# 101001000/ElevenRender

Hardware: AMD Instinct MI355X
Metric: Msamples/sec (rays traced x bounces) at 1920x1080, 1M-tri scene (higher is better)
Workload: dtype f32; 1 GPU; C2: 1000000-triangle random soup + 2048x1024 sky HDRI, 1920x1080, max_bounces 8, 1 step = 1 spp pass (config total 256 spp), seed 12345; schedule=stream

## Files before the change

### elevenrender_amd/abi.py

```python
import ctypes as C
import os

import numpy as np

_HERE = os.path.dirname(os.path.abspath(__file__))
LIB_PATH = os.environ.get("ELEVEN_HIP_LIB") or os.path.join(_HERE, "libeleven_hip.so")

ER_OK = 0
ER_ERR_INVALID_ARG, ER_ERR_NO_DEVICE, ER_ERR_HIP, ER_ERR_STATE, ER_ERR_OOM = -1, -2, -3, -4, -5
PASS_BEAUTY, PASS_DENOISE, PASS_NORMAL, PASS_TANGENT, PASS_BITANGENT, PASS_COUNT = 0, 1, 2, 3, 4, 5
PASS_NAMES = {"beauty": 0, "denoise": 1, "normal": 2, "tangent": 3, "bitangent": 4}
FLAG_POINT_LIGHTS, FLAG_COUNTERS, FLAG_MEGAKERNEL, FLAG_PROFILE, FLAG_FUSED, FLAG_WAVEFRONT, FLAG_GPU_BUILD, FLAG_MIS, FLAG_STREAM = 1, 2, 4, 8, 16, 32, 64, 128, 256
FLAG_HOST_BUILD = 512
FLAG_MESH_LIGHTS = 1024
UPDATE_CAMERA, UPDATE_GEOMETRY = 1, 2
EDIT_CAMERA, EDIT_GEOMETRY, EDIT_MATERIALS, EDIT_TEXTURES, EDIT_HDRI = 1, 2, 4, 8, 16
REBUILD_NEVER, REBUILD_ALWAYS, REBUILD_AUTO = 0, 1, 2
TOPO_REMOVE, TOPO_APPEND = 1, 2
FEATURE_ALBEDO, FEATURE_DEPTH, FEATURE_COUNT = 0, 1, 2
FEATURE_NAMES = {"albedo": 0, "depth": 1}
ID_NONE, ID_SLOTS = 0xFFFFFFFF, 4
ID_TRIANGLE, ID_OBJECT, ID_MATERIAL, ID_KIND_COUNT = 0, 1, 2, 3
ID_KIND_NAMES = {"triangle": 0, "object": 1, "material": 2}

# ... 491 lines not shown
    "er_state_import": (C.c_int, [_P, _P, C.c_uint64]),
    "er_comm_unique_id": (C.c_int, [C.POINTER(C.c_uint8)]),
    "er_comm_create": (C.c_int, [C.POINTER(C.c_uint8), C.c_uint32, C.c_uint32, C.c_int, C.POINTER(_P)]),
    "er_comm_destroy": (None, [_P]),
    "er_gather_pass": (C.c_int, [_P, C.c_int, _P, C.c_uint32]),
    "er_debug_comm_create_local": (C.c_int, [C.c_uint32, C.POINTER(_P)]),
    "er_comm_create_local": (C.c_int, [C.c_uint32, C.POINTER(_P)]),
    "er_debug_stream_info": (C.c_int, [_P, C.POINTER(ErStreamInfo)]),
    "er_debug_gather_buffers": (C.c_int, [_P, C.c_uint32, C.POINTER(_P), C.POINTER(C.c_uint64), C.POINTER(_P), C.POINTER(C.c_uint64)]),
    "er_debug_comm_loopback": (C.c_int, [_P, C.c_uint64, C.POINTER(C.c_double)]),
    "er_measure_hbm_peak": (C.c_int, [C.c_int, C.c_uint64, C.c_uint32, _FP, _FP]),
    "er_debug_eval": (C.c_int, [_P, C.c_int, _FP, C.c_uint32, C.c_uint32, _FP, C.c_uint32]),
    "er_debug_trace_rays": (C.c_int, [_P, _FP, _FP, C.c_uint32, _IP, _FP, _IP, _IP, _FP, _FP, _IP]),
    "er_debug_trace_pixel": (C.c_int, [_P, C.c_uint32, C.POINTER(ErTraceRec), C.c_int, C.POINTER(C.c_int)]),
    "er_debug_read_light_table": (C.c_int, [_P, _IP, _FP, C.c_uint32]),
    "er_debug_set_host_alloc_limit": (None, [C.c_uint64]),
    "er_debug_set_gpu_build_failure": (None, [C.c_int]),
    "er_debug_closest_hit": (C.c_int, [_P, C.POINTER(C.c_float), C.POINTER(C.c_float), C.c_uint32, C.POINTER(C.c_int32), C.POINTER(C.c_float),
                                       C.POINTER(C.c_float)]),
}

_lib = None


class ErError(RuntimeError):
    def __init__(self, code, msg):
        super().__init__(f"eleven_hip error {code}: {msg}")
        self.code = code


# ... 151 lines not shown
```

### elevenrender_amd/csrc/er_api.cpp

```cpp
#include <algorithm>
#include <chrono>

#include "er_api_stages.h"
#include <thread>
#include <system_error>

using namespace erh;

int er_abi_version(void) { return ER_ABI_VERSION; }
const char* er_last_error(void) { return g_err.c_str(); }

int er_device_count(void) {
    int n = 0;
    if (hipGetDeviceCount(&n) != hipSuccess) return 0;
    return n;
}

static int er_device_info_impl(int index, ErDeviceInfo* out) {
    if (!out) return fail(ER_ERR_INVALID_ARG, "er_device_info: out is NULL");
    int n = er_device_count();
    if (index < 0 || index >= n) return fail(ER_ERR_NO_DEVICE, "er_device_info: no such HIP device");
    hipDeviceProp_t p;
    HIP_TRY(hipGetDeviceProperties(&p, index));
    memset(out, 0, sizeof(*out));
// ... 316 lines not shown
            o[0] = a[0];
            o[1] = A.channels == 1 ? a[0] : a[1];
            o[2] = A.channels == 1 ? a[0] : (A.channels == 2 ? 0.0f : a[2]);
            o[3] = powered && !r_done ? ermath::er_pow(r, 2.2f) : r;
            o[4] = powered && !k_done ? ermath::er_pow(mt, 2.2f) : mt;
        }
    }
    s->fused_any = P.fused_any;
    if ((rc = upload(s->d_mat_fused, fused.data(), fused.size(), s->stream)) != ER_OK) return rc;
    s->kept.hdri = P.hdri;
    if (!s->hdri_tex.data.empty()) memcpy(pool.data() + P.hdri.offset, s->hdri_tex.data.data(), s->hdri_tex.data.size() * sizeof(float));
    if ((rc = upload(s->d_textures, table.data(), table.size(), s->stream)) != ER_OK) return rc;
    if ((rc = upload(s->d_tex_pool, pool.data(), pool.size(), s->stream)) != ER_OK) return rc;
    s->tex_pool_cap = pool.size();
    if ((rc = upload(s->d_cdf, s->hdri_cdf.data(), s->hdri_cdf.size(), s->stream)) != ER_OK) return rc;
    s->kept.buckets = er_build_cdf_guide(s->hdri_cdf.data(), s->hdri_tex.width * s->hdri_tex.height, B.guide);
    return upload(s->d_guide, B.guide.data(), B.guide.size(), s->stream);
}

int begin_emitters(ErScene* s, BeginStaging& B, const char* who) {
    if (!(s->params.flags & ER_FLAG_MESH_LIGHTS)) return ER_OK;
    int rc;
    std::vector<int32_t>& etex = B.etex;
    for (const ErMaterial& m : s->materials)
        if (m.emission_tex >= 0 && (size_t)m.emission_tex < s->textures.size()) etex.push_back(m.emission_tex);
    std::sort(etex.begin(), etex.end());
    etex.erase(std::unique(etex.begin(), etex.end()), etex.end());
    ScopedDevBuf<int32_t> d_etex;
    if ((rc = upload(d_etex, etex.data(), etex.size(), s->stream)) != ER_OK) return rc;
    float* tab = nullptr;
    HIP_TRY(er_lights_build(s->d_nodes8.p + s->kept.accel.n8_pieces, s->d_attr.p, s->tri_count, s->d_materials.p, s->d_textures.p, s->d_tex_pool.p, d_etex.p,
                            (uint32_t)etex.size(), (uint32_t)s->textures.size(), &tab, &s->light_emitters, &s->light_total, s->stream));
// ... 106 lines not shown
    D.node8_count = g.nodes8_count;
    D.prune_margin = lift_bound + 1e-5f * scene_scale;
    D.max_lift = lift_bound;
    D.scene_scale = scene_scale;
    D.materials = s->d_materials.p;
    D.mat_pre = s->d_mat_pre.p;
    D.textures = s->d_textures.p;
    D.tex_pool = s->d_tex_pool.p;
    D.mat_fused = s->d_mat_fused.p;
    D.fused_any = s->fused_any ? 1u : 0u;
    D.hdri_tex = s->kept.hdri;
    D.hdri_cdf = s->d_cdf.p;
    D.hdri_guide = s->d_guide.p;
    D.hdri_buckets = s->kept.buckets;
    D.hdri_radiance_sum = s->hdri_radiance_sum;
    D.cam = s->camera;
    D.x_res = s->x_res;
    D.y_res = s->y_res;
    D.tiles_x = s->tiles_x();
    D.tiles_y = s->tiles_y();
    D.max_bounces = s->params.max_bounces;
    {
        auto pow2 = [](int32_t v) { return v > 0 && (v & (v - 1)) == 0; };
        bool all = pow2(s->kept.hdri.width) && pow2(s->kept.hdri.height);
        for (const HostTex& t : s->textures) all = all && pow2(t.width) && pow2(t.height);
        D.tex_pow2 = all ? 1u : 0u;
        if (const char* e = getenv("ER_TEX_POW2")) D.tex_pow2 = (atoi(e) != 0 && all) ? 1u : 0u;
    }
    D.trace_every_query = 0u;
    if (const char* e = getenv("ER_TRACE_EVERY_QUERY")) D.trace_every_query = atoi(e) != 0 ? 1u : 0u;
// ... 620 lines not shown
```

### elevenrender_amd/csrc/er_api_edit.cpp

```cpp
#include <algorithm>
#include <chrono>

#include "er_api_stages.h"
#include "er_topology_host.h"

using namespace erh;

static_assert(ER_TOPO_REMOVE == ER_TOPO_HOST_REMOVE && ER_TOPO_APPEND == ER_TOPO_HOST_APPEND, "er_topology_host.h restates the two bits");

static_assert(ER_EDIT_CAMERA == ER_UPDATE_CAMERA && ER_EDIT_GEOMETRY == ER_UPDATE_GEOMETRY, "an ErSceneUpdate's bits are the first two of an ErSceneEdit");

namespace {

const uint32_t LOOK_BITS = ER_EDIT_MATERIALS | ER_EDIT_TEXTURES | ER_EDIT_HDRI;

struct XformList {
    uint32_t count = 0;
    const ErObjectTransform* x = nullptr;
    std::vector<ErXformEntry> entries;
    uint32_t moved = 0;
};


int edit_refit(ErScene* s, bool new_normals, bool new_tangents, const ErSparseList* sp, const XformList* xf, const char* who) {
// ... 202 lines not shown
            s->d_tex_pool.release();
            s->d_tex_pool = bigger;
            s->tex_pool_cap = std::max<size_t>(need, 1);
        }
        if (!s->hdri_tex.data.empty())
            HIP_TRY(hipMemcpyAsync(s->d_tex_pool.p + head, s->hdri_tex.data.data(), s->hdri_tex.data.size() * sizeof(float), hipMemcpyHostToDevice, s->stream));
        HIP_TRY(hipEventRecord(ev.b, s->stream));
        HIP_TRY(hipStreamSynchronize(s->stream));
        (void)hipEventElapsedTime(&stage_ms, ev.a, ev.b);
        s->d_tex_pool.n = need;
        s->kept.hdri = DevTex{s->hdri_tex.width, s->hdri_tex.height, s->hdri_tex.channels, s->hdri_tex.filter, (uint32_t)head};
        stage = 1;
    }
    if (what & ER_EDIT_HDRI) {
        if ((rc = upload(s->d_cdf, s->hdri_cdf.data(), s->hdri_cdf.size(), s->stream)) != ER_OK) return rc;
        s->kept.buckets = er_build_cdf_guide(s->hdri_cdf.data(), s->hdri_tex.width * s->hdri_tex.height, B.guide);
        if ((rc = upload(s->d_guide, B.guide.data(), B.guide.size(), s->stream)) != ER_OK) return rc;
    }
    return ER_OK;
}

int edit_emitters(ErScene* s, BeginStaging& B, const char* who) {
    s->d_light_tab.release(); s->light_emitters = 0; s->light_total = 0.0f;
    return begin_emitters(s, B, who);
}

int edit_restart(ErScene* s, BeginStaging& B) {
    s->ad_on = false;
    s->rendered = 0;
    s->timing_open = false;
    s->prof_used = 0;
    s->profile = ErProfile{};
// ... 480 lines not shown
```

### elevenrender_amd/csrc/er_api_stages.h

```cpp
#pragma once
#include "er_scene.h"

namespace erh {

struct BeginStaging {
    ErBvhBuild bvh;
    std::vector<ErTriIsect> isect;
    std::vector<ErTriAttr> attr;
    std::vector<float4> geom, mat_pre;
    std::vector<DevTex> table;
    std::vector<float> pool;
    std::vector<DevFused> fused;
    std::vector<uint32_t> guide, owned;
    std::vector<int32_t> etex;
    StreamDeal deal;
};

inline int check_pool_floats(uint64_t floats, const char* who) {
    return floats >= (1ull << 32) ? fail(ER_ERR_INVALID_ARG, std::string(who) + ": texture pool exceeds 2^32 floats") : ER_OK;
}

int begin_accel(ErScene* s, BeginStaging& B, hipEvent_t built_ev, const char* who, const ErGpuSceneArrays* device_arrays = nullptr);
bool accel_device_first(const ErScene* s);
void accel_publish(ErScene* s, float up_ms);
int upload_materials(ErScene* s, BeginStaging& B);
void plan_of_scene(const ErScene* s, TexPlan& P);
int begin_emitters(ErScene* s, BeginStaging& B, const char* who);
int begin_render_state(ErScene* s, BeginStaging& B, hipEvent_t uploads_done);

}
```

### elevenrender_amd/csrc/er_bounce.inc

```
#ifndef ER_BOUNCE_FUSE
#define ER_BOUNCE_FUSE true
#endif
#ifndef ER_BOUNCE_SKIP_EQUAL
#define ER_BOUNCE_SKIP_EQUAL true
#endif
{
    const bool er_skip_equal = (ER_BOUNCE_SKIP_EQUAL) && S.trace_every_query == 0u;
    const int hw = S.hdri_tex.width, hh = S.hdri_tex.height;
    const bool er_mis = EXT && (S.ext_flags & ER_FLAG_MIS) != 0;
#ifdef ER_BOUNCE_MESH
    constexpr bool er_mesh = EXT && (ER_BOUNCE_MESH);
#else
    constexpr bool er_mesh = false;
#endif
    if (hslot < 0) {
        float u, v;
        spherical_mapping(-1 * ray.d, u, v);
        if (EXT) {
            F3 er_env = tex_filtered(S, S.hdri_tex, u, v);
            if (er_mis && prev_pdf >= 0.0f) {
                const float er_ph = hdri_pdf(S, ermath::f2i(u * hw), ermath::f2i(v * hh));
                er_env = er_env * (1.0f / (1.0f + er_ph / prev_pdf));
                if (COUNT) c_texels++;
            }
            light = light + reduction * er_env;
        } else {
            light = light + reduction * tex_filtered(S, S.hdri_tex, u, v);
        }
        if (COUNT) c_texels++;
        done = true;
    } else {
        c_shaded++;
        ER_TP(2);
        HitFull hit;
        full_hit(S, (uint32_t)hslot, ray, hit);
        const ErMaterial& mat = S.materials[hit.material];
        HitData hd;
        generate_hit_data<COUNT, ER_BOUNCE_FUSE>(S, mat, hit, hd, c_texels);
        int shader = mat.albedo_shader_id;
        if (shader != -1) {
            hd.albedo = f3s(0);
            if (shader >= 0 && shader < 4) hd.albedo = f3(1, 1, 0);
        }
        if (rng_next(rs) <= hd.opacity) {
            F3 wo = ray.d * -1.0f;
            F3 N = hd.normal;
            c_hdri++;
            ER_TP(3);
            int count = er_cdf_search(S.hdri_cdf, hw * hh, S.hdri_guide, S.hdri_buckets, rng_next(rs));
            const bool hw_pow2 = (hw & (hw - 1)) == 0 && hw > 0 && count >= 0;
            float tcx = (float)(hw_pow2 ? (int)((unsigned)count & (unsigned)(hw - 1)) : count % hw);
            float tcy = (float)(hw_pow2 ? (int)((unsigned)count >> (31 - __builtin_clz((unsigned)hw))) : count / hw);
            float d1 = rng_next(rs), d2 = rng_next(rs), d3 = rng_next(rs);
            const bool er_lights = EXT && !er_mesh && (S.ext_flags & ER_FLAG_POINT_LIGHTS) != 0 && S.light_count > 0;
            float er_rl = 0.0f;
            if (er_lights) er_rl = rng_next(rs);
            float er_mp = 0.0f, er_mu1 = 0.0f, er_mu2 = 0.0f;
            if (er_mesh) { er_mp = rng_next(rs); er_mu1 = rng_next(rs); er_mu2 = rng_next(rs); }
            ER_TP(4);
            F3 wibrdf = DisneySample(hd, wo, N, d1, d2, d3);
            float nu = tcx / (float)hw, nv = tcy / (float)hh;
            float iu, iv;
            inverse_transform_uv(S.hdri_tex, nu, nv, iu, iv);
            F3 wihdri = normalized(reverse_spherical_mapping(iu, iv)) * -1.0f;
            F3 hdriValue = tex_uv(S, S.hdri_tex, iu, iv);
            if (COUNT) c_texels += 2;
            F3 evalh = DisneyEval(hd, wo, N, wihdri);
            float hdripdf = hdri_pdf(S, ermath::f2i(iu * hw), ermath::f2i(iv * hh));
            float absdot = __builtin_fabsf(dot(wihdri, N));
            float er_wnee = 1.0f;
            if (er_mis) er_wnee = 1.0f / (1.0f + DisneyPdf(hd, wo, N, wihdri) / hdripdf);
            F3 er_em = hd.emission;
            if (er_mesh && prev_pdf >= 0.0f) {
                const float er_ph = mesh_prob(S)[hslot];
                if (er_ph > 0.0f) {
                    F3 er_a, er_b, er_c, er_ng;
                    float er_area;
                    mesh_tri(S, (uint32_t)hslot, er_a, er_b, er_c, er_ng, er_area);
                    const float er_dh = mesh_d + length(hit.position - ray.o);
                    const float er_pl = er_ph * (er_dh * er_dh) / (er_area * __builtin_fabsf(dot(er_ng, ray.d)));
                    er_em = er_em * (1.0f / (1.0f + er_pl / prev_pdf));
                }
            }
// ... 65 lines not shown
                        const float er_lpdf = mesh_prob(S)[er_k] * (er_dist * er_dist) / (er_area * __builtin_fabsf(er_cosl));
                        const float er_wl = 1.0f / (1.0f + DisneyPdf(hd, wo, N, er_dir) / er_lpdf);
                        const F3 er_ml = er_le * er_evall * __builtin_fabsf(dot(er_dir, N)) / er_lpdf * er_wl;
                        const F3 er_lv = reduction * er_ml, er_lo = reduction * f3s(0);
                        if (er_skip_equal && !pending && same_bits(er_lv, er_lo)) {
                            light = light + er_lv;
                        } else {
                            const Ray er_lr = make_ray(hd.position + er_dir * 0.001f, er_dir);
                            ER_BOUNCE_LIGHT_QUERY(er_lr, (int)er_k, length(er_p - er_lr.o), er_lv, er_lo);
                            lpending = true;
                        }
                    }
                }
            }
            ER_TP(5);
            float brdfpdf = DisneyPdf(hd, wo, N, wibrdf);
            reduction = reduction * (DisneyEval(hd, wo, N, wibrdf) * __builtin_fabsf(dot(wibrdf, N)) / brdfpdf);
            if (er_mis || er_mesh) prev_pdf = brdfpdf;
            if (bounce == 0) { ER_BOUNCE_FIRST_HIT(hd.normal, hd.tangent, hd.bitangent); }
            ray = make_ray(hit.position + wibrdf * 0.001f, wibrdf);
            if (er_mesh) mesh_d = 0.001f;
        } else {
            if (er_mesh) mesh_d = mesh_d + length(hit.position - ray.o) + 0.001f;
            ray = make_ray(hit.position + ray.d * 0.001f, ray.d);
        }
        ER_TP(6);
        bounce++;
        if (bounce >= S.max_bounces) done = true;
    }
}
```

### elevenrender_amd/csrc/er_debug.hip

```cpp
#include "er_debug.h"

#include "er_device.h"
#include "er_shade.h"
#include "er_trav.h"

using namespace erd;

__global__ __launch_bounds__(64) void er_debug_trace_kernel(DevScene S, const float* __restrict__ o, const float* __restrict__ d, uint32_t n,
                                                             const int32_t* __restrict__ self, const float* __restrict__ limit,
                                                             int32_t* __restrict__ tri_out, int32_t* __restrict__ slot_out, float* __restrict__ pos_out,
                                                             float* __restrict__ dist_out, int32_t* __restrict__ info_out, uint2* spill_base) {
    __shared__ uint2 s_stack[WF_LDS_STACK * 64];
    __shared__ int s_stack2[ER_STACK * 64];
    const uint32_t i = blockIdx.x * 64 + threadIdx.x;
    if (i >= n) return;
    uint2* stack = s_stack + threadIdx.x;
    uint2* spill = spill_base + (size_t)blockIdx.x * (ER_STACK8 * 64) + threadIdx.x;
    int* stack2 = s_stack2 + threadIdx.x;
    Ray ray;
    ray.o = f3(o[3 * i], o[3 * i + 1], o[3 * i + 2]);
    ray.d = f3(d[3 * i], d[3 * i + 1], d[3 * i + 2]);
    unsigned cn = 0, ct = 0;
    int info = 0;
    if (self) {
// ... 75 lines not shown
            const int cs_ = trav_run_closest<false>(S, s_stack, spill, s_stack2, (sr), __builtin_inff(), info_, c_nodes, c_tris);     \
            rec->shadow_tri = cs_ < 0 ? -1 : __builtin_bit_cast(int, S.tri_isect[(size_t)cs_ * 3].w);                                 \
        }                                                                                                                             \
    }
#define ER_BOUNCE_LIGHT_QUERY(lr, self_slot, limit, lv, lo)                                                                          \
    {                                                                                                                                 \
        int info_;                                                                                                                    \
        c_rays++;                                                                                                                     \
        const bool occ_ = trav_run_shadow<false>(S, s_stack, spill, s_stack2, (lr), (self_slot), (limit), info_, c_nodes, c_tris);    \
        light = light + (occ_ ? (lo) : (lv));                                                                                         \
        if (rec) rec->light_occ = occ_ ? 1 : 0;                                                                                       \
    }
#define ER_BOUNCE_FIRST_HIT(n, t, b) aov_n = (n); aov_t = (t); aov_b = (b)
#define ER_BOUNCE_MESH MESH
#define ER_BOUNCE_SKIP_EQUAL false
#include "er_bounce.inc"
#undef ER_BOUNCE_HDRI_QUERY
#undef ER_BOUNCE_LIGHT_QUERY
#undef ER_BOUNCE_FIRST_HIT
#undef ER_BOUNCE_MESH
#undef ER_BOUNCE_SKIP_EQUAL
        (void)pending; (void)lpending; (void)traced;
        if (rec) {
            uint32_t r1 = rs_before;
            (void)rng_next(r1);
            rec->opaque = (hslot >= 0 && rs != r1) ? 1 : 0;
            if (hslot >= 0) { rec->wi[0] = ray.d.x; rec->wi[1] = ray.d.y; rec->wi[2] = ray.d.z; }
            rec->light[0] = light.x; rec->light[1] = light.y; rec->light[2] = light.z;
            rec->reduction[0] = reduction.x; rec->reduction[1] = reduction.y; rec->reduction[2] = reduction.z;
        }
        if (done) break;
    }
    const uint32_t sa = S.samples[idx];
    const uint32_t sa2 = accumulate_sample(S, idx, sa, light, aov_n, aov_t, aov_b);
    if (sa2 != sa) S.samples[idx] = sa2;
    S.rng[idx] = rs;
// ... 150 lines not shown
```

### elevenrender_amd/csrc/er_debug_api.cpp

```cpp
#include "er_scene.h"
#include "er_debug.h"

using namespace erh;

#include "../../include/eleven_hip_debug.h"

static int er_debug_closest_hit_impl(ErScene* s, const float* origins, const float* dirs, uint32_t n, int32_t* tri_ids, float* positions, float* distances) {
    if (!s || !origins || !dirs || !tri_ids || !positions || !distances) return fail(ER_ERR_INVALID_ARG, "er_debug_closest_hit: NULL argument");
    std::lock_guard<std::mutex> lk(s->mtx);
    if (!s->begun) return fail(ER_ERR_STATE, "er_debug_closest_hit: er_render_begin has not succeeded");
    HIP_TRY(hipSetDevice(s->device));
    ScopedDevBuf<float> d_o, d_d, d_pos, d_dist;
    ScopedDevBuf<int32_t> d_tri;
    int rc;
    if ((rc = upload(d_o, origins, (size_t)n * 3, s->stream)) != ER_OK) return rc;
    if ((rc = upload(d_d, dirs, (size_t)n * 3, s->stream)) != ER_OK) return rc;
    if ((rc = upload(d_pos, (const float*)nullptr, (size_t)n * 3, s->stream)) != ER_OK) return rc;
    if ((rc = upload(d_dist, (const float*)nullptr, (size_t)n, s->stream)) != ER_OK) return rc;
    if ((rc = upload(d_tri, (const int32_t*)nullptr, (size_t)n, s->stream)) != ER_OK) return rc;
    er_launch_debug_hit(s->dev, d_o.p, d_d.p, n, d_tri.p, d_pos.p, d_dist.p, s->stream);
    HIP_TRY(hipGetLastError());
    HIP_TRY(hipMemcpyAsync(tri_ids, d_tri.p, (size_t)n * 4, hipMemcpyDeviceToHost, s->stream));
    HIP_TRY(hipMemcpyAsync(positions, d_pos.p, (size_t)n * 12, hipMemcpyDeviceToHost, s->stream));
    HIP_TRY(hipMemcpyAsync(distances, d_dist.p, (size_t)n * 4, hipMemcpyDeviceToHost, s->stream));
// ... 355 lines not shown
    if (m == 0) return ER_OK;
    HIP_TRY(hipSetDevice(s->device));
    ScopedDevBuf<int32_t> d_tri;
    ScopedDevBuf<float> d_cdf;
    int rc;
    if ((rc = upload(d_tri, (const int32_t*)nullptr, m, s->stream)) != ER_OK) return rc;
    if ((rc = upload(d_cdf, (const float*)nullptr, m, s->stream)) != ER_OK) return rc;
    er_launch_light_table_read(s->dev.tri_isect, s->d_light_tab.p, s->tri_count, s->light_emitters, m, d_tri.p, d_cdf.p, s->stream);
    HIP_TRY(hipGetLastError());
    if (tri_index) HIP_TRY(hipMemcpyAsync(tri_index, d_tri.p, sizeof(int32_t) * m, hipMemcpyDeviceToHost, s->stream));
    if (cdf) HIP_TRY(hipMemcpyAsync(cdf, d_cdf.p, sizeof(float) * m, hipMemcpyDeviceToHost, s->stream));
    HIP_TRY(hipStreamSynchronize(s->stream));
    return ER_OK;
}

static int er_debug_eval_impl(ErScene* s, int kind, const float* in, uint32_t n, uint32_t in_stride, float* out, uint32_t out_stride) {
    static const uint32_t need_in[ER_FN_COUNT] = {1, 7, 7, 29, 29, 29, 3, 2, 4, 1, 2, 3};
    static const uint32_t need_out[ER_FN_COUNT] = {32, 6, 18, 3, 1, 3, 2, 3, 3, 1, 1, 1};
    if (!s || !in || !out) return fail(ER_ERR_INVALID_ARG, "er_debug_eval: NULL argument");
    if (kind < 0 || kind >= ER_FN_COUNT) return fail(ER_ERR_INVALID_ARG, "er_debug_eval: unknown kind");
    if (in_stride < need_in[kind] || out_stride < need_out[kind]) return fail(ER_ERR_INVALID_ARG, "er_debug_eval: stride smaller than the kind's item");
    std::lock_guard<std::mutex> lk(s->mtx);
    if (!s->begun) return fail(ER_ERR_STATE, "er_debug_eval: er_render_begin has not succeeded");
    if (kind == ER_FN_TEXTURE)
        for (uint32_t i = 0; i < n; i++) {
            int32_t id;
            memcpy(&id, &in[(size_t)i * in_stride], 4);
            if (id < -1 || id >= (int32_t)s->textures.size()) return fail(ER_ERR_INVALID_ARG, "er_debug_eval: texture id out of range");
            if (id >= 0 && (size_t)id < s->tex_mode.size() && s->tex_mode[(size_t)id] != 0)
                return fail(ER_ERR_STATE, "er_debug_eval: texture " + std::to_string(id) + " is kept compacted on the device (first channel" +
// ... 110 lines not shown
    return guarded("er_debug_accel_cost_host", [&]() -> int {
        return er_debug_accel_cost_host_impl(nodes8, node8_count, node8_pieces, isect, tri_count, sums, node_terms, node_cap, tri_terms, tri_cap);
    });
}
int er_debug_bvh_check(const float* vertices, const float* normals, uint32_t tri_count, int threads, ErBvhCheck* out) { return guarded("er_debug_bvh_check", [&]() -> int { return er_debug_bvh_check_impl(vertices, normals, tri_count, threads, out); }); }
int er_debug_trace_rays(ErScene* s, const float* origins, const float* dirs, uint32_t n, const int32_t* self_slots, const float* limits, int32_t* tri_ids,
                        int32_t* slots, float* positions, float* distances, int32_t* info) {
    return guarded("er_debug_trace_rays", [&]() -> int { return er_debug_trace_rays_impl(s, origins, dirs, n, self_slots, limits, tri_ids, slots, positions, distances, info); });
}
int er_debug_trace_pixel(ErScene* s, uint32_t idx, ErTraceRec* recs, int max_recs, int* count) {
    return guarded("er_debug_trace_pixel", [&]() -> int { return er_debug_trace_pixel_impl(s, idx, recs, max_recs, count); });
}
int er_debug_read_light_table(ErScene* s, int32_t* tri_index, float* cdf, uint32_t cap) {
    return guarded("er_debug_read_light_table", [&]() -> int { return er_debug_read_light_table_impl(s, tri_index, cdf, cap); });
}
int er_debug_eval(ErScene* s, int kind, const float* in, uint32_t n, uint32_t in_stride, float* out, uint32_t out_stride) {
    return guarded("er_debug_eval", [&]() -> int { return er_debug_eval_impl(s, kind, in, n, in_stride, out, out_stride); });
}
int er_measure_hbm_peak(int device, uint64_t bytes, uint32_t iters, float* copy_GBps, float* read_GBps) {
    return guarded("er_measure_hbm_peak", [&]() -> int { return er_measure_hbm_peak_impl(device, bytes, iters, copy_GBps, read_GBps); });
}
int er_debug_transform_apply(const float* m, uint32_t count, const float* v, const float* n, const float* t, float* ov, float* on, float* ot) {
    return guarded("er_debug_transform_apply", [&]() -> int {
        if (!m || (count && (!v || !n || !t || !ov || !on || !ot))) return fail(ER_ERR_INVALID_ARG, "er_debug_transform_apply: NULL argument");
        if (!er_xform_apply(m, count, v, n, t, ov, on, ot)) return fail(ER_ERR_INVALID_ARG, "er_debug_transform_apply: a matrix entry is not finite, or det(L) is not > 0");
        return ER_OK;
    });
}
int er_debug_id_rank(const uint32_t* ids, uint32_t count, uint32_t* out_ids, uint32_t* out_counts, uint32_t* distinct) {
    return guarded("er_debug_id_rank", [&]() -> int {
// ... 8 lines not shown
```

### elevenrender_amd/csrc/er_device.h

```cpp
#pragma once
#include <hip/hip_runtime.h>
#include <stdint.h>

#include "../../include/eleven_hip.h"
#include "er_bvh.h"
#include "er_cdf.h"
#include "er_math.h"

#ifdef ER_ISA_MARKS
#define ER_MARK(name) asm volatile("; ER_MARK " name ::: "memory")
#else
#define ER_MARK(name) ((void)0)
#endif

#ifndef ER_TP
#define ER_TP(n) ((void)0)
#endif

#define ER_TILE 8
#define ER_STACK ER_BVH_MAX_DEPTH

struct DevTex {
    int32_t width, height, channels, filter;
    uint32_t offset;
// ... 36 lines not shown
    uint32_t tex_pow2;
    float cam_cx, cam_sx, cam_cy, cam_sy, cam_cz, cam_sz;
    uint32_t cam_trig_valid;
    uint32_t trace_every_query;
    uint32_t ext_flags;
    union { const ErPointLight* lights; const float* mesh_lights; };
    union { uint32_t light_count; uint32_t emitter_count; };
    float4* passes;
    uint32_t* samples;
    uint32_t* rng;
    const uint32_t* owned_tiles;
    uint32_t owned_tile_count;
    DevCounters* counters;
    uint32_t* tile_cost;
    uint32_t* px_draws;
};

__host__ __device__ __forceinline__ size_t er_pass_index(size_t npx, int pass, size_t idx) {
    return pass == ER_PASS_DENOISE ? 4 * npx + idx : idx * 4 + (size_t)(pass == ER_PASS_BEAUTY ? 0 : pass - 1);
}


namespace erd {

#define ERD __device__ __forceinline__

const float PIF = 3.14159265358979323846f;

struct F3 { float x, y, z; };
ERD F3 f3(float x, float y, float z) { F3 r; r.x = x; r.y = y; r.z = z; return r; }
// ... 12 lines not shown
ERD float dot(F3 a, F3 b) { return a.x * b.x + a.y * b.y + a.z * b.z; }
ERD F3 cross(F3 a, F3 b) {
    return f3((a.y * b.z - a.z * b.y), -(a.x * b.z - a.z * b.x), (a.x * b.y - a.y * b.x));
}
ERD float length(F3 a) { return __builtin_sqrtf(a.x * a.x + a.y * a.y + a.z * a.z); }
ERD F3 normalized(F3 a) {
    float l = length(a);
    if (l == 0) return a;
    return a / l;
}
ERD float clampf(float a, float b, float c) { return a < b ? b : a > c ? c : a; }
ERD float lerpf(float a, float b, float c) { return a + c * (b - a); }
ERD F3 lerpv(F3 a, F3 b, float c) { return f3(lerpf(a.x, b.x, c), lerpf(a.y, b.y, c), lerpf(a.z, b.z, c)); }
ERD float minf(float a, float b) { return a < b ? a : b; }
ERD float maxf(float a, float b) { return a > b ? a : b; }
ERD void limitUV(float& u, float& v) {
    u += (float)(-(int)(u > 1) + -(int)(u < 0));
    v += (float)(-(int)(v > 1) + -(int)(v < 0));
}

struct Ray { F3 o, d; };
ERD Ray make_ray(F3 o, F3 d) {
    Ray r;
    r.o = o;
    float l = length(d);
    if (l != 0) { d.x /= l; d.y /= l; d.z /= l; }
    r.d = d;
    return r;
}

ERD uint32_t jenkins_u32(uint32_t seed) {
// ... 284 lines not shown
        fused_coords(S, t, ermath::f2i(t2x), ermath::f2i(t2y), a4, r4);
        alb = lerpv(lerpv(a1, a2, a), lerpv(a3, a4, a), b);
        rm = lerpv(lerpv(r1, r2, a), lerpv(r3, r4, a), b);
    } else {
        fused_coords(S, t, ermath::f2i(u * t.width), ermath::f2i(v * t.height), alb, rm);
    }
}
ERD void spherical_mapping(F3 point, float& u, float& v) {
    F3 p = (point - f3s(0)) / 1.0f;
    float theta = ermath::er_acos(-p.y);
    float phi = ermath::er_atan2(-p.z, p.x) + PIF;
    u = phi / (2 * PIF);
    v = theta / PIF;
    limitUV(u, v);
}
ERD void inverse_transform_uv(const DevTex& t, float u, float v, float& nu, float& nv) {
    int x = ermath::f2i(u * t.width);
    int y = ermath::f2i(v * t.height);
    nu = (float)x / (float)t.width;
    nv = (float)y / (float)t.height;
    limitUV(nu, nv);
}
ERD F3 reverse_spherical_mapping(float u, float v) {
    float phi = u * 2 * PIF;
    float theta = v * PIF;
    float px = ermath::er_cos(phi - PIF);
    float py = -ermath::er_cos(theta);
    float pz = -ermath::er_sin(phi - PIF);
    float a = __builtin_sqrtf(1 - py * py);
    return f3(a * px, py, a * pz);
}

ERD int hdri_binary_search(const float* arr, float value, int length) {
    int from = 0;
    int to = length - 1;
    while (to - from > 0) {
        int m = from + (to - from) / 2;
        if (m >= length || m < 0) return 0;
        float am = arr[m];
        if (value == am) return m;
        if (value < am) to = m - 1;
        if (value > am) from = m + 1;
    }
    return to;
}
ERD float hdri_pdf(const DevScene& S, int x, int y) {
    F3 dv = tex_coords(S, S.hdri_tex, x, y);
    float theta = (((float)y / (float)S.hdri_tex.height)) * PIF;
    return ((dv.x + dv.y + dv.z) / S.hdri_radiance_sum) * S.hdri_tex.width * S.hdri_tex.height / (2.0f * PIF * ermath::er_sin(theta));
}

struct HitData {
    float metallic, roughness, clearcoatGloss, clearcoat, anisotropic, transmission, specular,
        specularTint, sheenTint, subsurface, sheen, opacity;
    float gtr1_log;
    F3 emission, albedo;
    F3 position, normal, tangent, bitangent;
};

ERD float SchlickFresnel(float u) {
    float m = clampf(1.0f - u, 0.0f, 1.0f);
    float m2 = m * m;
    return m2 * m2 * m;
}
// ... 159 lines not shown
```

### elevenrender_amd/csrc/er_scene.h

```cpp
#pragma once
#include <hip/hip_runtime.h>

#include <atomic>
#include <cmath>
#include <cstdio>
#include <cstdlib>
#include <cstring>
#include <map>
#include <set>
#include <memory>
#include <mutex>
#include <new>
#include <string>
#include <vector>

#include "../../include/eleven_hip.h"
#include "er_bvh.h"
#include "er_devbuf.h"
#include "er_device.h"
#include "er_gpu_build.h"
#include "er_kernels.h"
#include "er_wavefront.h"
#include "er_stream.h"
#include "er_stream_host.h"
// ... 116 lines not shown

    bool begun = false;
    int device = 0;
    ErRenderParams params{};
    hipStream_t stream = nullptr;
    hipEvent_t ev_start = nullptr, ev_stop = nullptr;
    bool timing_open = false;
    DevScene dev{};
    ErAccelInfo accel{};
    float accel_lo[3] = {0, 0, 0}, accel_hi[3] = {0, 0, 0};
    uint32_t accel_depth2 = 0;
    struct Kept {
        ErGpuBvhDevice accel;
        DevTex hdri{};
        int buckets = 0;
        uint32_t cus = 0, flags = 0;
    } kept;
    ErRefitTopo refit_topo;
    ErUpdateInfo upd{};
    ErEditInfo edit{};
    ErSparseInfo sparse{};
    ErObjectTable objects;
    ErXformDev xform_dev;
    ErSparseInfo xform{};
    uint32_t xform_objects = 0;
    ErGeomStore store;
    ErTopologyInfo topo{};
    void flush_poses() noexcept { er_objects_flush(objects, vertices.data(), normals.data(), tangents.data()); }
    uint64_t accel_version = 0, cost_version = ~0ull;
    ErAccelCost cost_kept{};
// ... 186 lines not shown
```

### elevenrender_amd/csrc/er_shade.h

```cpp
#pragma once
#include "er_device.h"

namespace erd {

static inline bool er_mesh_active(const DevScene& S) { return (S.ext_flags & ER_FLAG_MESH_LIGHTS) != 0; }
static inline bool er_ext_active(const DevScene& S) {
    return (S.ext_flags & ER_FLAG_MIS) != 0 || ((S.ext_flags & ER_FLAG_POINT_LIGHTS) != 0 && S.light_count > 0) || er_mesh_active(S);
}

ERD const float* mesh_prob(const DevScene& S) { return S.mesh_lights; }
ERD const float* mesh_cdf(const DevScene& S) { return S.mesh_lights + S.tri_count; }
ERD uint32_t mesh_slot(const DevScene& S, uint32_t k) { return __builtin_bit_cast(uint32_t, S.mesh_lights[(size_t)S.tri_count + S.emitter_count + k]); }
ERD uint32_t mesh_pick(const DevScene& S, float r) {
    const float* cdf = mesh_cdf(S);
    uint32_t lo = 0, hi = S.emitter_count;
    while (lo < hi) {
        const uint32_t m = lo + ((hi - lo) >> 1);
        if (cdf[m] > r) hi = m; else lo = m + 1;
    }
    return lo < S.emitter_count ? lo : S.emitter_count - 1;
}
ERD void mesh_tri(const DevScene& S, uint32_t slot, F3& v0, F3& v1, F3& v2, F3& ng, float& area) {
    float4 a, b, c;
    load_verts(S, slot, v0, v1, v2, a, b, c);
// ... 29 lines not shown
```

### elevenrender_amd/render.py

```python
import ctypes as C
from dataclasses import dataclass

import numpy as np

from . import abi, topology as topo


@dataclass
class RenderParameters:
    width: int = 1280
    height: int = 720
    sampleTarget: int = 100
    denoise: bool = False
    device: str = ""
    block_size: int = 8
    max_bounces: int = 5
    rank: int = 0
    world: int = 1
    flags: int = 0


@dataclass
class RenderInfo:
    samples: int = 0
# ... 332 lines not shown
        return {n: getattr(a, n) for n, _ in abi.ErAdaptiveInfo._fields_}

    def light_info(self):
        li = abi.ErLightInfo()
        abi.check(self.lib.er_light_info(self.handle, C.byref(li)))
        return {n: getattr(li, n) for n, _ in abi.ErLightInfo._fields_}

    def debug_light_table(self):
        n = self.light_info()["emitters"]
        tri = np.zeros(n, np.int32)
        cdf = np.zeros(n, np.float32)
        if n:
            abi.check(self.lib.er_debug_read_light_table(self.handle, tri.ctypes.data_as(C.POINTER(C.c_int32)), cdf.ctypes.data_as(C.POINTER(C.c_float)), n))
        return tri, cdf

    def tile_state(self):
        tx, ty = (self.scene.x_res + 7) // 8, (self.scene.y_res + 7) // 8
        err = np.empty((ty, tx), np.float32)
        spp = np.empty((ty, tx), np.uint32)
        abi.check(self.lib.er_read_tile_state(self.handle, err.ctypes.data_as(C.POINTER(C.c_float)), spp.ctypes.data_as(C.POINTER(C.c_uint32))))
        return err, spp

    def denoise(self, levels=0, colour_sigma=0.0):
        abi.check(self.lib.er_denoise(self.handle, levels, colour_sigma))

    def render_features(self, n=0):
        abi.check(self.lib.er_render_features(self.handle, n))

    def get_feature(self, name):
        f = abi.FEATURE_NAMES[str(name).lower()]
# ... 221 lines not shown
```

### include/eleven_hip_debug.h

```cpp
#ifndef ELEVEN_HIP_DEBUG_H
#define ELEVEN_HIP_DEBUG_H
#include <stdint.h>
#ifdef __cplusplus
extern "C" {
#endif

typedef struct ErBvhCheck {
    uint32_t node_count, leaf_count, max_depth, max_leaf_size;
    uint32_t tris_in_leaves;
    uint32_t duplicate_tris;
    uint32_t uncontained;
    uint32_t unreachable_nodes;
    float lift_bound;
    float build_ms;
    double sah_cost;
} ErBvhCheck;

int er_debug_bvh_check(const float* vertices, const float* normals, uint32_t tri_count, int threads, ErBvhCheck* out);

typedef struct ErAccelDump {
    uint32_t tri_count;
    uint32_t node_count;
    uint32_t node8_count;
    uint32_t node8_pieces;
// ... 33 lines not shown
    int32_t bounce;
    int32_t tri;
    int32_t shadow_tri;
    int32_t opaque;
    float position[3];
    float wi[3];
    float light[3];
    float reduction[3];
    int32_t shadow_occ;
    int32_t light_occ;
} ErTraceRec;

int er_debug_trace_pixel(struct ErScene* scene, uint32_t idx, ErTraceRec* recs, int max_recs, int* count);

int er_debug_read_light_table(struct ErScene* scene, int32_t* tri_index, float* cdf, uint32_t cap);

enum { ER_FN_RNG = 0, ER_FN_CAMERA_RAY, ER_FN_TRI_HIT, ER_FN_DISNEY_EVAL, ER_FN_DISNEY_PDF, ER_FN_DISNEY_SAMPLE, ER_FN_SPHERICAL,
       ER_FN_REV_SPHERICAL, ER_FN_TEXTURE, ER_FN_HDRI_SEARCH, ER_FN_HDRI_PDF, ER_FN_MATH, ER_FN_COUNT };
int er_debug_eval(struct ErScene* scene, int kind, const float* in, uint32_t n, uint32_t in_stride, float* out, uint32_t out_stride);

struct ErComm;
int er_debug_comm_create_local(uint32_t world, struct ErComm** out);

typedef struct ErStreamInfo {
    uint32_t waves, tracers;
    uint32_t large_regions;
    uint32_t deal_pending;
    uint32_t launches;
    uint32_t pixels_per_cu;
    double lanes_busy;
// ... 92 lines not shown
```

Measured before the change: 2109 Msamples/s.

## Precompute HDRI per-row/column trig tables and skip BRDF sampling on last bounce

Adds a small device table of per-column (cos/sin of phi, texel index) and per-row (cos theta, sqrt, sine pdf) values for the HDRI. NEE light sampling and the MIS pdf now look these up instead of evaluating sin/cos per sample. It also reuses the sampled HDRI texel value for the pdf instead of fetching it twice. A third change skips DisneySample, DisneyPdf, DisneyEval and the next-ray setup on the final bounce, since that ray is never traced. The costs are an extra table load per sample and slightly different float paths.

```diff
diff --git a/elevenrender_amd/abi.py b/elevenrender_amd/abi.py
--- a/elevenrender_amd/abi.py
+++ b/elevenrender_amd/abi.py
@@ -529,6 +529,8 @@
     "er_debug_trace_rays": (C.c_int, [_P, _FP, _FP, C.c_uint32, _IP, _FP, _IP, _IP, _FP, _FP, _IP]),
     "er_debug_trace_pixel": (C.c_int, [_P, C.c_uint32, C.POINTER(ErTraceRec), C.c_int, C.POINTER(C.c_int)]),
     "er_debug_read_light_table": (C.c_int, [_P, _IP, _FP, C.c_uint32]),
+    "er_debug_read_hdri_trig": (C.c_int, [_P, _UP, C.c_uint32, _UP, C.c_uint32]),
+    "er_debug_hdri_trig_host": (C.c_int, [C.c_int32, C.c_int32, _UP, _UP]),
     "er_debug_set_host_alloc_limit": (None, [C.c_uint64]),
     "er_debug_set_gpu_build_failure": (None, [C.c_int]),
     "er_debug_closest_hit": (C.c_int, [_P, C.POINTER(C.c_float), C.POINTER(C.c_float), C.c_uint32, C.POINTER(C.c_int32), C.POINTER(C.c_float),
diff --git a/elevenrender_amd/csrc/er_api.cpp b/elevenrender_amd/csrc/er_api.cpp
--- a/elevenrender_amd/csrc/er_api.cpp
+++ b/elevenrender_amd/csrc/er_api.cpp
@@ -354,8 +354,19 @@
     if ((rc = upload(s->d_tex_pool, pool.data(), pool.size(), s->stream)) != ER_OK) return rc;
     s->tex_pool_cap = pool.size();
     if ((rc = upload(s->d_cdf, s->hdri_cdf.data(), s->hdri_cdf.size(), s->stream)) != ER_OK) return rc;
+    return upload_hdri_guide(s, B);
+}
+
+int upload_hdri_guide(ErScene* s, BeginStaging& B) {
+    int rc;
     s->kept.buckets = er_build_cdf_guide(s->hdri_cdf.data(), s->hdri_tex.width * s->hdri_tex.height, B.guide);
-    return upload(s->d_guide, B.guide.data(), B.guide.size(), s->stream);
+    const size_t at = (B.guide.size() + 3) & ~(size_t)3;
+    B.guide.resize(at + erd::hdri_trig_words(s->kept.hdri.width, s->kept.hdri.height), 0u);
+    if ((rc = upload(s->d_guide, B.guide.data(), B.guide.size(), s->stream)) != ER_OK) return rc;
+    s->kept.trig_at = at;
+    er_launch_hdri_trig(s->kept.hdri, s->d_guide.p + at, s->stream);
+    HIP_TRY(hipGetLastError());
+    return ER_OK;
 }
 
 int begin_emitters(ErScene* s, BeginStaging& B, const char* who) {
@@ -492,6 +503,7 @@
     D.hdri_guide = s->d_guide.p;
     D.hdri_buckets = s->kept.buckets;
     D.hdri_radiance_sum = s->hdri_radiance_sum;
+    D.hdri_trig = getenv("ER_HDRI_TRIG_ON_DEVICE") ? nullptr : s->d_guide.p + s->kept.trig_at;
     D.cam = s->camera;
     D.x_res = s->x_res;
     D.y_res = s->y_res;
diff --git a/elevenrender_amd/csrc/er_api_edit.cpp b/elevenrender_amd/csrc/er_api_edit.cpp
--- a/elevenrender_amd/csrc/er_api_edit.cpp
+++ b/elevenrender_amd/csrc/er_api_edit.cpp
@@ -240,8 +240,7 @@
     }
     if (what & ER_EDIT_HDRI) {
         if ((rc = upload(s->d_cdf, s->hdri_cdf.data(), s->hdri_cdf.size(), s->stream)) != ER_OK) return rc;
-        s->kept.buckets = er_build_cdf_guide(s->hdri_cdf.data(), s->hdri_tex.width * s->hdri_tex.height, B.guide);
-        if ((rc = upload(s->d_guide, B.guide.data(), B.guide.size(), s->stream)) != ER_OK) return rc;
+        if ((rc = upload_hdri_guide(s, B)) != ER_OK) return rc;
     }
     return ER_OK;
 }
diff --git a/elevenrender_amd/csrc/er_api_stages.h b/elevenrender_amd/csrc/er_api_stages.h
--- a/elevenrender_amd/csrc/er_api_stages.h
+++ b/elevenrender_amd/csrc/er_api_stages.h
@@ -1,5 +1,6 @@
 #pragma once
 #include "er_scene.h"
+#include "er_hdri_trig.h"
 
 namespace erh {
 
@@ -24,6 +25,7 @@
 bool accel_device_first(const ErScene* s);
 void accel_publish(ErScene* s, float up_ms);
 int upload_materials(ErScene* s, BeginStaging& B);
+int upload_hdri_guide(ErScene* s, BeginStaging& B);
 void plan_of_scene(const ErScene* s, TexPlan& P);
 int begin_emitters(ErScene* s, BeginStaging& B, const char* who);
 int begin_render_state(ErScene* s, BeginStaging& B, hipEvent_t uploads_done);
diff --git a/elevenrender_amd/csrc/er_bounce.inc b/elevenrender_amd/csrc/er_bounce.inc
--- a/elevenrender_amd/csrc/er_bounce.inc
+++ b/elevenrender_amd/csrc/er_bounce.inc
@@ -3,6 +3,9 @@
 #endif
 #ifndef ER_BOUNCE_SKIP_EQUAL
 #define ER_BOUNCE_SKIP_EQUAL true
+#endif
+#ifndef ER_BOUNCE_KEEP_LAST
+#define ER_BOUNCE_KEEP_LAST false
 #endif
 {
     const bool er_skip_equal = (ER_BOUNCE_SKIP_EQUAL) && S.trace_every_query == 0u;
@@ -19,7 +22,9 @@
         if (EXT) {
             F3 er_env = tex_filtered(S, S.hdri_tex, u, v);
             if (er_mis && prev_pdf >= 0.0f) {
-                const float er_ph = hdri_pdf(S, ermath::f2i(u * hw), ermath::f2i(v * hh));
+                const int er_mx = ermath::f2i(u * hw), er_my = ermath::f2i(v * hh);
+                const float er_ms = (S.hdri_trig != nullptr && (unsigned)er_my < (unsigned)hh) ? hdri_trig_rows(S)[er_my].sin_row : hdri_pdf_sine(S.hdri_tex, er_my);
+                const float er_ph = hdri_pdf_of(S, tex_coords(S, S.hdri_tex, er_mx, er_my), er_ms);
                 er_env = er_env * (1.0f / (1.0f + er_ph / prev_pdf));
                 if (COUNT) c_texels++;
             }
@@ -49,8 +54,9 @@
             ER_TP(3);
             int count = er_cdf_search(S.hdri_cdf, hw * hh, S.hdri_guide, S.hdri_buckets, rng_next(rs));
             const bool hw_pow2 = (hw & (hw - 1)) == 0 && hw > 0 && count >= 0;
-            float tcx = (float)(hw_pow2 ? (int)((unsigned)count & (unsigned)(hw - 1)) : count % hw);
-            float tcy = (float)(hw_pow2 ? (int)((unsigned)count >> (31 - __builtin_clz((unsigned)hw))) : count / hw);
+            const int er_cx = hw_pow2 ? (int)((unsigned)count & (unsigned)(hw - 1)) : count % hw;
+            const int er_cy = hw_pow2 ? (int)((unsigned)count >> (31 - __builtin_clz((unsigned)hw))) : count / hw;
+            float tcx = (float)er_cx, tcy = (float)er_cy;
             float d1 = rng_next(rs), d2 = rng_next(rs), d3 = rng_next(rs);
             const bool er_lights = EXT && !er_mesh && (S.ext_flags & ER_FLAG_POINT_LIGHTS) != 0 && S.light_count > 0;
             float er_rl = 0.0f;
@@ -58,15 +64,30 @@
             float er_mp = 0.0f, er_mu1 = 0.0f, er_mu2 = 0.0f;
             if (er_mesh) { er_mp = rng_next(rs); er_mu1 = rng_next(rs); er_mu2 = rng_next(rs); }
             ER_TP(4);
-            F3 wibrdf = DisneySample(hd, wo, N, d1, d2, d3);
-            float nu = tcx / (float)hw, nv = tcy / (float)hh;
-            float iu, iv;
-            inverse_transform_uv(S.hdri_tex, nu, nv, iu, iv);
-            F3 wihdri = normalized(reverse_spherical_mapping(iu, iv)) * -1.0f;
-            F3 hdriValue = tex_uv(S, S.hdri_tex, iu, iv);
+            const bool er_last = !(ER_BOUNCE_KEEP_LAST) && bounce + 1u >= S.max_bounces;
+            F3 wibrdf = f3s(0);
+            if (!er_last) wibrdf = DisneySample(hd, wo, N, d1, d2, d3);
+            float er_px, er_pz, er_py, er_a, er_sin;
+            int er_ix, er_iy;
+            if (S.hdri_trig != nullptr && (unsigned)count < (unsigned)(hw * hh)) {
+                const HdriCol er_c = hdri_trig_cols(S)[er_cx];
+                const HdriRow er_r = hdri_trig_rows(S)[er_cy];
+                er_px = er_c.px; er_pz = er_c.pz; er_ix = er_c.ix;
+                er_py = er_r.py; er_a = er_r.a; er_iy = er_r.iy; er_sin = er_r.sin_pdf;
+            } else {
+                float nu = tcx / (float)hw, nv = tcy / (float)hh;
+                float iu, iv;
+                inverse_transform_uv(S.hdri_tex, nu, nv, iu, iv);
+                rsm_column(iu, er_px, er_pz);
+                rsm_row(iv, er_py, er_a);
+                er_ix = ermath::f2i(iu * hw); er_iy = ermath::f2i(iv * hh);
+                er_sin = hdri_pdf_sine(S.hdri_tex, er_iy);
+            }
+            F3 wihdri = normalized(f3(er_a * er_px, er_py, er_a * er_pz)) * -1.0f;
+            F3 hdriValue = tex_coords(S, S.hdri_tex, er_ix, er_iy);
             if (COUNT) c_texels += 2;
             F3 evalh = DisneyEval(hd, wo, N, wihdri);
-            float hdripdf = hdri_pdf(S, ermath::f2i(iu * hw), ermath::f2i(iv * hh));
+            float hdripdf = hdri_pdf_of(S, hdriValue, er_sin);
             float absdot = __builtin_fabsf(dot(wihdri, N));
             float er_wnee = 1.0f;
             if (er_mis) er_wnee = 1.0f / (1.0f + DisneyPdf(hd, wo, N, wihdri) / hdripdf);
@@ -162,11 +183,13 @@
                 }
             }
             ER_TP(5);
-            float brdfpdf = DisneyPdf(hd, wo, N, wibrdf);
-            reduction = reduction * (DisneyEval(hd, wo, N, wibrdf) * __builtin_fabsf(dot(wibrdf, N)) / brdfpdf);
-            if (er_mis || er_mesh) prev_pdf = brdfpdf;
+            if (!er_last) {
+                float brdfpdf = DisneyPdf(hd, wo, N, wibrdf);
+                reduction = reduction * (DisneyEval(hd, wo, N, wibrdf) * __builtin_fabsf(dot(wibrdf, N)) / brdfpdf);
+                if (er_mis || er_mesh) prev_pdf = brdfpdf;
+                ray = make_ray(hit.position + wibrdf * 0.001f, wibrdf);
+            }
             if (bounce == 0) { ER_BOUNCE_FIRST_HIT(hd.normal, hd.tangent, hd.bitangent); }
-            ray = make_ray(hit.position + wibrdf * 0.001f, wibrdf);
             if (er_mesh) mesh_d = 0.001f;
         } else {
             if (er_mesh) mesh_d = mesh_d + length(hit.position - ray.o) + 0.001f;
diff --git a/elevenrender_amd/csrc/er_debug.hip b/elevenrender_amd/csrc/er_debug.hip
--- a/elevenrender_amd/csrc/er_debug.hip
+++ b/elevenrender_amd/csrc/er_debug.hip
@@ -113,12 +113,14 @@
 #define ER_BOUNCE_FIRST_HIT(n, t, b) aov_n = (n); aov_t = (t); aov_b = (b)
 #define ER_BOUNCE_MESH MESH
 #define ER_BOUNCE_SKIP_EQUAL false
+#define ER_BOUNCE_KEEP_LAST true
 #include "er_bounce.inc"
 #undef ER_BOUNCE_HDRI_QUERY
 #undef ER_BOUNCE_LIGHT_QUERY
 #undef ER_BOUNCE_FIRST_HIT
 #undef ER_BOUNCE_MESH
 #undef ER_BOUNCE_SKIP_EQUAL
+#undef ER_BOUNCE_KEEP_LAST
         (void)pending; (void)lpending; (void)traced;
         if (rec) {
             uint32_t r1 = rs_before;
diff --git a/elevenrender_amd/csrc/er_debug_api.cpp b/elevenrender_amd/csrc/er_debug_api.cpp
--- a/elevenrender_amd/csrc/er_debug_api.cpp
+++ b/elevenrender_amd/csrc/er_debug_api.cpp
@@ -1,5 +1,6 @@
 #include "er_scene.h"
 #include "er_debug.h"
+#include "er_hdri_trig.h"
 
 using namespace erh;
 
@@ -393,6 +394,29 @@
     return ER_OK;
 }
 
+static int er_debug_read_hdri_trig_impl(ErScene* s, uint32_t* cols, uint32_t col_cap, uint32_t* rows, uint32_t row_cap) {
+    if (!s) return fail(ER_ERR_INVALID_ARG, "er_debug_read_hdri_trig: NULL scene");
+    std::lock_guard<std::mutex> lk(s->mtx);
+    if (!s->begun) return fail(ER_ERR_STATE, "er_debug_read_hdri_trig: er_render_begin has not succeeded");
+    const DevTex& t = s->kept.hdri;
+    const size_t nc = std::min<size_t>(col_cap, (size_t)std::max(t.width, 0)), nr = std::min<size_t>(row_cap, (size_t)std::max(t.height, 0));
+    HIP_TRY(hipSetDevice(s->device));
+    const uint32_t* tab = s->d_guide.p + s->kept.trig_at;
+    if (cols && nc) HIP_TRY(hipMemcpyAsync(cols, tab, nc * sizeof(erd::HdriCol), hipMemcpyDeviceToHost, s->stream));
+    if (rows && nr) HIP_TRY(hipMemcpyAsync(rows, tab + erd::hdri_trig_row_offset(t.width), nr * sizeof(erd::HdriRow), hipMemcpyDeviceToHost, s->stream));
+    HIP_TRY(hipStreamSynchronize(s->stream));
+    return ER_OK;
+}
+
+static int er_debug_hdri_trig_host_impl(int32_t width, int32_t height, uint32_t* cols, uint32_t* rows) {
+    if (width < 0 || height < 0 || (width && !cols) || (height && !rows)) return fail(ER_ERR_INVALID_ARG, "er_debug_hdri_trig_host: bad argument");
+    std::vector<uint32_t> tab(erd::hdri_trig_words(width, height));
+    er_hdri_trig_host(DevTex{width, height, 3, 0, 0u}, tab.data());
+    if (width) memcpy(cols, tab.data(), (size_t)width * sizeof(erd::HdriCol));
+    if (height) memcpy(rows, tab.data() + erd::hdri_trig_row_offset(width), (size_t)height * sizeof(erd::HdriRow));
+    return ER_OK;
+}
+
 static int er_debug_eval_impl(ErScene* s, int kind, const float* in, uint32_t n, uint32_t in_stride, float* out, uint32_t out_stride) {
     static const uint32_t need_in[ER_FN_COUNT] = {1, 7, 7, 29, 29, 29, 3, 2, 4, 1, 2, 3};
     static const uint32_t need_out[ER_FN_COUNT] = {32, 6, 18, 3, 1, 3, 2, 3, 3, 1, 1, 1};
@@ -533,6 +557,12 @@
 int er_debug_read_light_table(ErScene* s, int32_t* tri_index, float* cdf, uint32_t cap) {
     return guarded("er_debug_read_light_table", [&]() -> int { return er_debug_read_light_table_impl(s, tri_index, cdf, cap); });
 }
+int er_debug_read_hdri_trig(ErScene* s, uint32_t* cols, uint32_t col_cap, uint32_t* rows, uint32_t row_cap) {
+    return guarded("er_debug_read_hdri_trig", [&]() -> int { return er_debug_read_hdri_trig_impl(s, cols, col_cap, rows, row_cap); });
+}
+int er_debug_hdri_trig_host(int32_t width, int32_t height, uint32_t* cols, uint32_t* rows) {
+    return guarded("er_debug_hdri_trig_host", [&]() -> int { return er_debug_hdri_trig_host_impl(width, height, cols, rows); });
+}
 int er_debug_eval(ErScene* s, int kind, const float* in, uint32_t n, uint32_t in_stride, float* out, uint32_t out_stride) {
     return guarded("er_debug_eval", [&]() -> int { return er_debug_eval_impl(s, kind, in, n, in_stride, out, out_stride); });
 }
diff --git a/elevenrender_amd/csrc/er_device.h b/elevenrender_amd/csrc/er_device.h
--- a/elevenrender_amd/csrc/er_device.h
+++ b/elevenrender_amd/csrc/er_device.h
@@ -74,6 +74,7 @@
     DevCounters* counters;
     uint32_t* tile_cost;
     uint32_t* px_draws;
+    const uint32_t* hdri_trig;
 };
 
 __host__ __device__ __forceinline__ size_t er_pass_index(size_t npx, int pass, size_t idx) {
@@ -116,7 +117,7 @@
 ERD F3 lerpv(F3 a, F3 b, float c) { return f3(lerpf(a.x, b.x, c), lerpf(a.y, b.y, c), lerpf(a.z, b.z, c)); }
 ERD float minf(float a, float b) { return a < b ? a : b; }
 ERD float maxf(float a, float b) { return a > b ? a : b; }
-ERD void limitUV(float& u, float& v) {
+__host__ __device__ __forceinline__ void limitUV(float& u, float& v) {
     u += (float)(-(int)(u > 1) + -(int)(u < 0));
     v += (float)(-(int)(v > 1) + -(int)(v < 0));
 }
@@ -431,20 +432,27 @@
     v = theta / PIF;
     limitUV(u, v);
 }
-ERD void inverse_transform_uv(const DevTex& t, float u, float v, float& nu, float& nv) {
+__host__ __device__ __forceinline__ void inverse_transform_uv(const DevTex& t, float u, float v, float& nu, float& nv) {
     int x = ermath::f2i(u * t.width);
     int y = ermath::f2i(v * t.height);
     nu = (float)x / (float)t.width;
     nv = (float)y / (float)t.height;
     limitUV(nu, nv);
 }
+__host__ __device__ __forceinline__ void rsm_column(float u, float& px, float& pz) {
+    float phi = u * 2 * PIF;
+    px = ermath::er_cos(phi - PIF);
+    pz = -ermath::er_sin(phi - PIF);
+}
+__host__ __device__ __forceinline__ void rsm_row(float v, float& py, float& a) {
+    float theta = v * PIF;
+    py = -ermath::er_cos(theta);
+    a = __builtin_sqrtf(1 - py * py);
+}
 ERD F3 reverse_spherical_mapping(float u, float v) {
-    float phi = u * 2 * PIF;
-    float theta = v * PIF;
-    float px = ermath::er_cos(phi - PIF);
-    float py = -ermath::er_cos(theta);
-    float pz = -ermath::er_sin(phi - PIF);
-    float a = __builtin_sqrtf(1 - py * py);
+    float px, py, pz, a;
+    rsm_column(u, px, pz);
+    rsm_row(v, py, a);
     return f3(a * px, py, a * pz);
 }
 
@@ -461,10 +469,16 @@
     }
     return to;
 }
+__host__ __device__ __forceinline__ float hdri_pdf_sine(const DevTex& t, int y) {
+    float theta = (((float)y / (float)t.height)) * PIF;
+    return ermath::er_sin(theta);
+}
+ERD float hdri_pdf_of(const DevScene& S, F3 dv, float sin_theta) {
+    return ((dv.x + dv.y + dv.z) / S.hdri_radiance_sum) * S.hdri_tex.width * S.hdri_tex.height / (2.0f * PIF * sin_theta);
+}
 ERD float hdri_pdf(const DevScene& S, int x, int y) {
     F3 dv = tex_coords(S, S.hdri_tex, x, y);
-    float theta = (((float)y / (float)S.hdri_tex.height)) * PIF;
-    return ((dv.x + dv.y + dv.z) / S.hdri_radiance_sum) * S.hdri_tex.width * S.hdri_tex.height / (2.0f * PIF * ermath::er_sin(theta));
+    return hdri_pdf_of(S, dv, hdri_pdf_sine(S.hdri_tex, y));
 }
 
 struct HitData {
diff --git a/elevenrender_amd/csrc/er_hdri_trig.h b/elevenrender_amd/csrc/er_hdri_trig.h
--- /dev/null
+++ b/elevenrender_amd/csrc/er_hdri_trig.h
@@ -0,0 +1,50 @@
+#pragma once
+#include "er_device.h"
+
+namespace erd {
+
+struct HdriCol {
+    float px, pz;
+    int32_t ix;
+    float iu;
+};
+struct HdriRow {
+    float py, a;
+    int32_t iy;
+    float sin_pdf;
+    float iv;
+    float sin_row;
+};
+static_assert(sizeof(HdriCol) == 16 && sizeof(HdriRow) == 24, "er_hdri_trig.h: table entry sizes");
+
+#define ER_HT_HD __host__ __device__ __forceinline__
+
+ER_HT_HD HdriCol hdri_col_entry(const DevTex& t, int x) {
+    HdriCol c;
+    float nu = (float)x / (float)t.width, iv;
+    inverse_transform_uv(t, nu, 0.0f, c.iu, iv);
+    rsm_column(c.iu, c.px, c.pz);
+    c.ix = ermath::f2i(c.iu * t.width);
+    return c;
+}
+ER_HT_HD HdriRow hdri_row_entry(const DevTex& t, int y) {
+    HdriRow r;
+    float nv = (float)y / (float)t.height, iu;
+    inverse_transform_uv(t, 0.0f, nv, iu, r.iv);
+    rsm_row(r.iv, r.py, r.a);
+    r.iy = ermath::f2i(r.iv * t.height);
+    r.sin_pdf = hdri_pdf_sine(t, r.iy);
+    r.sin_row = hdri_pdf_sine(t, y);
+    return r;
+}
+
+ER_HT_HD size_t hdri_trig_row_offset(int width) { return (size_t)(width > 0 ? width : 0) * 4; }
+ER_HT_HD size_t hdri_trig_words(int width, int height) { return hdri_trig_row_offset(width) + (size_t)(height > 0 ? height : 0) * 6; }
+
+__device__ __forceinline__ const HdriCol* hdri_trig_cols(const DevScene& S) { return (const HdriCol*)S.hdri_trig; }
+__device__ __forceinline__ const HdriRow* hdri_trig_rows(const DevScene& S) { return (const HdriRow*)(S.hdri_trig + hdri_trig_row_offset(S.hdri_tex.width)); }
+
+}
+
+void er_launch_hdri_trig(const DevTex& t, uint32_t* table, hipStream_t stream);
+void er_hdri_trig_host(const DevTex& t, uint32_t* table);
diff --git a/elevenrender_amd/csrc/er_hdri_trig.hip b/elevenrender_amd/csrc/er_hdri_trig.hip
--- /dev/null
+++ b/elevenrender_amd/csrc/er_hdri_trig.hip
@@ -0,0 +1,26 @@
+#include "er_hdri_trig.h"
+
+using namespace erd;
+
+__global__ __launch_bounds__(64) void er_hdri_trig_kernel(DevTex t, uint32_t* __restrict__ table) {
+    const int w = t.width > 0 ? t.width : 0, h = t.height > 0 ? t.height : 0;
+    const int i = (int)(blockIdx.x * 64u + threadIdx.x);
+    if (i < w) {
+        ((HdriCol*)table)[i] = hdri_col_entry(t, i);
+    } else if (i - w < h) {
+        ((HdriRow*)(table + hdri_trig_row_offset(t.width)))[i - w] = hdri_row_entry(t, i - w);
+    }
+}
+
+void er_launch_hdri_trig(const DevTex& t, uint32_t* table, hipStream_t stream) {
+    const long long n = (long long)(t.width > 0 ? t.width : 0) + (long long)(t.height > 0 ? t.height : 0);
+    if (n == 0) return;
+    hipLaunchKernelGGL(er_hdri_trig_kernel, dim3((unsigned)((n + 63) / 64)), dim3(64), 0, stream, t, table);
+}
+
+void er_hdri_trig_host(const DevTex& t, uint32_t* table) {
+    HdriCol* cols = (HdriCol*)table;
+    HdriRow* rows = (HdriRow*)(table + hdri_trig_row_offset(t.width));
+    for (int x = 0; x < t.width; x++) cols[x] = hdri_col_entry(t, x);
+    for (int y = 0; y < t.height; y++) rows[y] = hdri_row_entry(t, y);
+}
diff --git a/elevenrender_amd/csrc/er_scene.h b/elevenrender_amd/csrc/er_scene.h
--- a/elevenrender_amd/csrc/er_scene.h
+++ b/elevenrender_amd/csrc/er_scene.h
@@ -154,6 +154,7 @@
         ErGpuBvhDevice accel;
         DevTex hdri{};
         int buckets = 0;
+        size_t trig_at = 0;
         uint32_t cus = 0, flags = 0;
     } kept;
     ErRefitTopo refit_topo;
diff --git a/elevenrender_amd/csrc/er_shade.h b/elevenrender_amd/csrc/er_shade.h
--- a/elevenrender_amd/csrc/er_shade.h
+++ b/elevenrender_amd/csrc/er_shade.h
@@ -1,5 +1,6 @@
 #pragma once
 #include "er_device.h"
+#include "er_hdri_trig.h"
 
 namespace erd {
 
diff --git a/elevenrender_amd/render.py b/elevenrender_amd/render.py
--- a/elevenrender_amd/render.py
+++ b/elevenrender_amd/render.py
@@ -370,6 +370,13 @@
             abi.check(self.lib.er_debug_read_light_table(self.handle, tri.ctypes.data_as(C.POINTER(C.c_int32)), cdf.ctypes.data_as(C.POINTER(C.c_float)), n))
         return tri, cdf
 
+    def debug_hdri_trig(self, width, height):
+        cols = np.zeros((width, 4), np.uint32)
+        rows = np.zeros((height, 6), np.uint32)
+        up = C.POINTER(C.c_uint32)
+        abi.check(self.lib.er_debug_read_hdri_trig(self.handle, cols.ctypes.data_as(up), width, rows.ctypes.data_as(up), height))
+        return cols, rows
+
     def tile_state(self):
         tx, ty = (self.scene.x_res + 7) // 8, (self.scene.y_res + 7) // 8
         err = np.empty((ty, tx), np.float32)
diff --git a/include/eleven_hip_debug.h b/include/eleven_hip_debug.h
--- a/include/eleven_hip_debug.h
+++ b/include/eleven_hip_debug.h
@@ -71,6 +71,9 @@
 int er_debug_trace_pixel(struct ErScene* scene, uint32_t idx, ErTraceRec* recs, int max_recs, int* count);
 
 int er_debug_read_light_table(struct ErScene* scene, int32_t* tri_index, float* cdf, uint32_t cap);
+
+int er_debug_read_hdri_trig(struct ErScene* scene, uint32_t* cols, uint32_t col_cap, uint32_t* rows, uint32_t row_cap);
+int er_debug_hdri_trig_host(int32_t width, int32_t height, uint32_t* cols, uint32_t* rows);
 
 enum { ER_FN_RNG = 0, ER_FN_CAMERA_RAY, ER_FN_TRI_HIT, ER_FN_DISNEY_EVAL, ER_FN_DISNEY_PDF, ER_FN_DISNEY_SAMPLE, ER_FN_SPHERICAL,
        ER_FN_REV_SPHERICAL, ER_FN_TEXTURE, ER_FN_HDRI_SEARCH, ER_FN_HDRI_PDF, ER_FN_MATH, ER_FN_COUNT };
```

Measured after the change: 2145 Msamples/s (median of 6 runs). 1.02x the previous value.
